# laurabragagnolo/SkelSplat

Measured on AMD Instinct MI355X. Metric: rendered+backpropagated views/s (differentiable skeletal-Gaussian rasterizer fwd+bwd), higher is better.
Workload: dtype f32

## Files before the change

### include/skelsplat_hip.h

```cpp
#ifndef SKELSPLAT_HIP_H
#define SKELSPLAT_HIP_H

#include <stddef.h>
#include <stdint.h>

#ifdef __cplusplus
extern "C" {
#endif

#define SKS_MAX_VIEWS 64
#define SKS_MAX_CHANNELS 32
#define SKS_SMALL_P 256

#define SKS_ANTIALIASING 1u
#define SKS_CLAMP01      2u
#define SKS_FORCE_BINNED 4u
#define SKS_DEBUG_SYNC   8u

#define SKS_NO_NT_STORES 16u

#define SKS_RAW_PARAMS   32u
#define SKS_RAW_GRADS    128u
#define SKS_BIN_CLEAN    64u
#define SKS_BIN_GROUPS_SHIFT 16
#define SKS_BIN_GROUPS(n) ((unsigned)(((n) - 1) & 7) << SKS_BIN_GROUPS_SHIFT)
#define SKS_FILL_LINEAR (1u << 21)
#define SKS_FILL_ROWS (1u << 22)
#define SKS_BWD_LDS_LIST (1u << 20)
#define SKS_BWD_WG_SHIFT 23

const char* sks_last_error(void);
int sks_version(void);

int sks_scratch_bytes(int V, int P, int C, int W, int H, size_t bin_capacity,
                      size_t* geom_bytes, size_t* binning_bytes, size_t* accum_bytes);

int sks_forward(int V, int P, int C, int W, int H,
                const float* viewmatrix, const float* projmatrix,
                const float* tanfovx , const float* tanfovy ,
                const float* means3D, const float* features, const float* opacities,
                const float* scales, const float* rotations, const float* cov3D_precomp,
                float scale_modifier, unsigned flags,
                float* out_color, float* out_invdepth, int* radii,
                void* geom, void* binning, size_t bin_capacity, int* num_rendered_dev,
                float* final_T, uint32_t* n_contrib, void* stream);

int sks_backward(int V, int P, int C, int W, int H,
                 const float* viewmatrix, const float* projmatrix,
                 const float* tanfovx , const float* tanfovy ,
                 const float* bg,
                 const float* means3D, const float* features, const float* opacities,
                 const float* scales, const float* rotations, const float* cov3D_precomp,
                 float scale_modifier, unsigned flags,
                 const int* radii, const void* geom, const void* binning, size_t bin_capacity,
                 const float* dL_dout_color, const float* dL_dout_invdepth,
                 void* accum,
                 float* dL_dmeans3D, float* dL_dmeans2D, float* dL_dopacity,
                 float* dL_dscales, float* dL_drotations, float* dL_dcov3D, float* dL_dfeatures,
                 float* dL_dmeans3D_mean ,
                 void* stream);

#define SKS_FB_NO_JOIN 1u
// ... 189 lines not shown
```

### skelsplat_amd/_lib.py

```python
import ctypes as C
import os

_HERE = os.path.dirname(os.path.abspath(__file__))
LIB_PATH = os.path.join(_HERE, "libskelsplat_hip.so")
_lib = None

SKS_MAX_VIEWS = 64
SKS_MAX_CHANNELS = 32
SKS_SMALL_P = 256
SKS_ANTIALIASING = 1
SKS_CLAMP01 = 2
SKS_FORCE_BINNED = 4
SKS_DEBUG_SYNC = 8
SKS_NO_NT_STORES = 16
SKS_RAW_PARAMS = 32
SKS_BIN_CLEAN = 64
SKS_RAW_GRADS = 128
SKS_FB_NO_JOIN = 1
SKS_BIN_GROUPS_SHIFT = 16
SKS_SSIM_SCRATCH_BYTES = 64 * 8
SKS_SOFTARGMAX_STATS = 6
SKS_REPORT_MAX_SAVES = 8
SKS_EVAL_MAX_GROUPS = 64


def SKS_BIN_GROUPS(n):
    return ((int(n) - 1) & 7) << SKS_BIN_GROUPS_SHIFT


_vp, _i, _u, _f, _sz = C.c_void_p, C.c_int, C.c_uint, C.c_float, C.c_size_t

_CAMERAS = (("V", _i), ("P", _i), ("C", _i), ("W", _i), ("H", _i), ("viewmatrix", _vp), ("projmatrix", _vp),
            ("tanfovx", _vp), ("tanfovy", _vp))
_GAUSSIANS = (("means3D", _vp), ("features", _vp), ("opacities", _vp), ("scales", _vp), ("rotations", _vp),
              ("cov3D_precomp", _vp), ("scale_modifier", _f), ("flags", _u))
_UPSTREAM = (("dL_dout_color", _vp), ("dL_dout_invdepth", _vp), ("accum", _vp))
_GRADS = (("dL_dmeans3D", _vp), ("dL_dmeans2D", _vp), ("dL_dopacity", _vp), ("dL_dscales", _vp), ("dL_drotations", _vp),
          ("dL_dcov3D", _vp), ("dL_dfeatures", _vp), ("dL_dmeans3D_mean", _vp))
_FORWARD_IO = (("out_color", _vp), ("out_invdepth", _vp), ("radii", _vp), ("geom", _vp), ("binning", _vp),
               ("bin_capacity", _sz), ("num_rendered_dev", _vp))
FORWARD_PARAMS = _CAMERAS + _GAUSSIANS + _FORWARD_IO + (("final_T", _vp), ("n_contrib", _vp), ("stream", _vp))
BACKWARD_PARAMS = _CAMERAS + (("bg", _vp),) + _GAUSSIANS + (("radii", _vp), ("geom", _vp), ("binning", _vp), ("bin_capacity", _sz)) \
    + _UPSTREAM + _GRADS + (("stream", _vp),)
FORWARD_BACKWARD_PARAMS = _CAMERAS + _GAUSSIANS + _FORWARD_IO + (("bg", _vp),) + _UPSTREAM + _GRADS \
    + (("stream", _vp), ("aux_stream", _vp), ("fb_flags", _u))

FWD, BWD, FWD_BWD = ({name: i for i, (name, _) in enumerate(params)}
                     for params in (FORWARD_PARAMS, BACKWARD_PARAMS, FORWARD_BACKWARD_PARAMS))
FWD_BWD_SOURCES = tuple(("fwd", FWD[n]) if n in FWD else ("bwd", BWD[n]) if n in BWD else None for n in FWD_BWD)

_ull = C.c_ulonglong
_VIEWS_DV = (("viewmatrix", _vp), ("projmatrix", _vp), ("views_dev", _vp))
RIG_SELECT_PARAMS = (("R", _i), ("V", _i), ("frames", _i), ("rig_ids", _vp), ("bank_viewmatrix", _vp), ("bank_projmatrix", _vp),
                     ("bank_tan", _vp), ("slot_wh", _vp), ("bank_proj", _vp), ("bank_sched", _vp), ("viewmatrix", _vp),
                     ("projmatrix", _vp), ("views_dev", _vp), ("proj", _vp), ("lr_sched_dev", _vp), ("error_word", _vp),
                     ("stream", _vp))
# ... 147 lines not shown
```

### skelsplat_amd/csrc/sks_common.inc

```
thread_local char g_err[512] = "";

int fail(int code, const char* fmt, ...)
{
    va_list ap;
    va_start(ap, fmt);
    vsnprintf(g_err, sizeof(g_err), fmt, ap);
    va_end(ap);
    return code;
}

#define HIP_TRY(expr)                                                                          \
    do {                                                                                       \
        hipError_t e_ = (expr);                                                                \
        if (e_ != hipSuccess) return fail((int)e_, "%s: %s", #expr, hipGetErrorString(e_));    \
    } while (0)

#define STAGE_CHECK(name)                                                                      \
    do {                                                                                       \
        HIP_TRY(hipGetLastError());                                                            \
        if (flags & SKS_DEBUG_SYNC) {                                                          \
            hipError_t e_ = hipStreamSynchronize(st);                                          \
            if (e_ != hipSuccess) return fail((int)e_, "stage %s: %s", name, hipGetErrorString(e_)); \
        }                                                                                      \
    } while (0)

constexpr int PROF_MAX = 16384;
struct ProfKind {
    hipEvent_t b[PROF_MAX], e[PROF_MAX];
    int created = 0, n = 0;
};
struct ProfState {
    bool on = false;
    int every = 1;
    int skip = 0;
    bool recorded = false;
    int seen[2] = { 0, 0 };
    ProfKind kind[2];
};
thread_local ProfState* tl_prof = nullptr;

struct ProfScope {
    ProfKind* k = nullptr;
    hipStream_t st;
    bool ext;
    ProfScope(int kind, hipStream_t s, bool ext_ = false) : st(s), ext(ext_)
    {
        ProfState* ps = tl_prof;
        if (!ps || !ps->on || ((ps->skip >> kind) & 1)) return;
        if (ps->seen[kind]++ % ps->every != 0) return;
        ProfKind& p = ps->kind[kind];
        if (p.n >= PROF_MAX) return;
        if (p.n >= p.created) {
            if (hipEventCreate(&p.b[p.created]) != hipSuccess || hipEventCreate(&p.e[p.created]) != hipSuccess) return;
            p.created++;
        }
        k = &p;
        if (ps->recorded) ext = false;
        if (!ext) (void)hipEventRecord(p.b[p.n], st);
    }
    hipEvent_t eb() const { return k->b[k->n]; }
    hipEvent_t ee() const { return k->e[k->n]; }
    ~ProfScope()
    {
        if (!k) return;
        if (!ext) (void)hipEventRecord(k->e[k->n], st);
        k->n++;
    }
};
#define SKS_LAUNCH(prof, kernel, grid, block, lds, stream, ...)                                                  \
    do {                                                                                                         \
        if ((prof).k) hipExtLaunchKernelGGL(kernel, grid, block, lds, stream, (prof).eb(), (prof).ee(), 0, __VA_ARGS__); \
        else hipLaunchKernelGGL(kernel, grid, block, lds, stream, __VA_ARGS__);                                  \
    } while (0)

constexpr int NACC = 8;
constexpr int BWD_SPLITS = 16;
constexpr int BWD_WG_PAIRS16 = 400;
constexpr int BWD_WG_PAIRS8 = 4096;

struct ViewTan {
    float x[SKS_MAX_VIEWS];
    float y[SKS_MAX_VIEWS];
    int w[SKS_MAX_VIEWS];
    int h[SKS_MAX_VIEWS];
};
struct ViewOff {
    unsigned long long off[SKS_MAX_VIEWS];
};
struct ViewTanDev {
    const float* x;
    const float* y;
    const int* w;
    const int* h;
    const double* sched;
};
inline ViewTanDev views_dev_from(const void* views_dev, const double* sched = nullptr)
{
    const ViewTan* t = (const ViewTan*)views_dev;
    return ViewTanDev{ t->x, t->y, t->w, t->h, sched };
}
inline bool fill_views(ViewTan& vt, ViewOff* vo, int V, int C, int W, int H, const float* tanfovx, const float* tanfovy,
                       const int* view_wh, const size_t* plane_off)
{
    for (int v = 0; v < V; v++) {
        vt.x[v] = tanfovx[v];
// ... 154 lines not shown
```

### skelsplat_amd/csrc/sks_fwd_small.inc

```
__device__ __forceinline__ float clamp01(float x) { return fminf(fmaxf(x, 0.0f), 1.0f); }

struct FwdArgs {
    int P, C, W, H;
    unsigned flags;
    Geom g;
    const float* features;
    float* out_color;
    float* out_invdepth;
    float* final_T;
    uint32_t* n_contrib;
    int tslots;
    unsigned cp1_magic;
    int ncomp;
    int cover_planes;
    unsigned w_magic;
};

inline int composite_slots(unsigned flags, int V, int P)
{
    const int t = (int)((flags >> 26) & 15u);
    return t ? t : ((long long)V * P <= 128 ? 4 : 8);
}

typedef float v4f __attribute__((ext_vector_type(4)));
// ... 5 lines not shown
__device__ __forceinline__ void store4(float* p, float a, float b, float c, float d)
{
    v4f v = { a, b, c, d };
    if (NT) __builtin_nontemporal_store(v, reinterpret_cast<v4f*>(p));
    else *reinterpret_cast<v4f*>(p) = v;
}
template <bool NT>
__device__ __forceinline__ void store2(float* p, float a, float b)
{
    v2f v = { a, b };
    if (NT) __builtin_nontemporal_store(v, reinterpret_cast<v2f*>(p));
    else *reinterpret_cast<v2f*>(p) = v;
}

template <int CG>
struct DynList {
    float2* xy;
    float4* co;
    float* invd;
    float* feat;
    unsigned long long* key;
    uint4* rect;
    __device__ DynList(char* base, int cap)
    {
        co = (float4*)base; base += (size_t)cap * 16;
        rect = (uint4*)base; base += (size_t)cap * 16;
        key = (unsigned long long*)base; base += (size_t)cap * 8;
        xy = (float2*)base; base += (size_t)cap * 8;
        invd = (float*)base; base += (size_t)cap * 4;
        feat = (float*)base;
    }
    static size_t bytes(int cap, int cg) { return (size_t)cap * (16 + 16 + 8 + 8 + 4 + 4 * (size_t)cg); }
};

template <int PPT, bool NT, bool HALF = false>
__device__ __forceinline__ void fwd_fill_role(const FwdArgs& a, unsigned cp1_magic, int q, int band, int zid, int gy, int pb,
                                              const uint32_t* __restrict__ cover)
{
    const int tid = threadIdx.x;
    const int P = a.P, C = a.C, W = a.W, H = a.H;
    const size_t HW = (size_t)H * W;
    const int v = (int)(((unsigned)zid * cp1_magic) >> 20);
    const int plane = zid - v * (C + 1);
    const bool is_inv = plane == C;
    const int cw = cover_cw(W);
    constexpr int PASS = 256 * PPT;
    const int rows = min(TILE, H - band * TILE);
    const int Nb = rows * W;
    const size_t band0 = (size_t)band * TILE * W;
    float* out = (is_inv ? a.out_invdepth + (size_t)v * HW : a.out_color + ((size_t)v * C + plane) * HW) + band0;
    const int shift = (int)((reinterpret_cast<uintptr_t>(out) >> 2) & 31u);
    const int base0 = q * PASS * pb + tid * PPT - shift;
    float* outT = (is_inv && a.final_T) ? a.final_T + (size_t)v * HW + band0 : nullptr;
    uint32_t* outN = (is_inv && a.n_contrib) ? a.n_contrib + (size_t)v * HW + band0 : nullptr;
    const uint32_t* __restrict__ cwp = cover;
    v4u c0 = { 0u, 0u, 0u, 0u }, c1 = { 0u, 0u, 0u, 0u };
    if (cover) {
        const int wo = __builtin_amdgcn_readfirstlane(((a.cover_planes ? zid : v) * gy + band) * cw);
        cwp = cover + wo;
        c0 = *reinterpret_cast<const v4u*>(cwp);
        if (cw > 4) c1 = *reinterpret_cast<const v4u*>(cwp + 4);
    }
    const bool any = c0.x != 0u;
    const unsigned w_magic = a.w_magic;
    auto mod_w = [&](int base) -> int {
        if (w_magic) return base - (int)__umulhi((unsigned)base, w_magic) * W;
        return base % W;
    };
    auto cover_word = [&](int wi) -> uint32_t {
        if (cw <= 4) return wi == 0 ? c0.y : wi == 1 ? c0.z : c0.w;
        if (cw <= 8) return wi == 0 ? c0.y : wi == 1 ? c0.z : wi == 2 ? c0.w : wi == 3 ? c1.x : wi == 4 ? c1.y : wi == 5 ? c1.z : c1.w;
        return cwp[1 + wi];
    };
    if (pb < 0) {
        const int pbr = -pb;
        const int chunks = (W + PASS - 1) / PASS;
        const int rb = q / chunks, chunk = q - rb * chunks;
        const int x = chunk * PASS + tid * PPT;
        if (x >= W) return;
        if (any) {
            const int tx = x >> 4;
            if ((cover_word(tx >> 5) >> (tx & 31)) & 1u) return;
        }
        const int r1 = min(rows, (rb + 1) * pbr);
        for (int r = rb * pbr; r < r1; r++) {
            const int base = r * W + x;
            store4<NT>(out + base, 0.0f, 0.0f, 0.0f, 0.0f);
            if (outT || outN) {
#pragma unroll
                for (int p = 0; p < PPT; p++) {
                    if (outT) outT[base + p] = 1.0f;
                    if (outN) outN[base + p] = 0u;
                }
            }
        }
        return;
    }
    const int npass = min(pb, 32);
    if (cover && !any) {
        for (int k = 0; k < npass; k++) {
            const int base = base0 + k * PASS;
            if (base >= Nb) break;
            if (base < 0) continue;
            if (PPT == 4) store4<NT>(out + base, 0.0f, 0.0f, 0.0f, 0.0f);
            else out[base] = 0.0f;
            if (outT || outN) {
#pragma unroll
                for (int p = 0; p < PPT; p++) {
                    if (outT) outT[base + p] = 1.0f;
                    if (outN) outN[base + p] = 0u;
                }
            }
        }
        return;
    }
    unsigned skipmask = 0u, skipmask2 = 0u;
    auto second_tx = [&](int x0) -> int { const int x1 = x0 + 2; return (x1 >= W ? x1 - W : x1) >> 4; };
    if (any && cw <= 8) {
        for (int k = 0; k < npass; k++) {
            const int base = base0 + k * PASS;
            if (base >= Nb) break;
            if (base < 0) continue;
            const int x0 = mod_w(base);
            const int tx = x0 >> 4;
            const bool s0 = (cover_word(tx >> 5) >> (tx & 31)) & 1u;
            bool s1 = s0;
            if (HALF) {
                const int tx1 = second_tx(x0);
                s1 = ((cover_word(tx1 >> 5) >> (tx1 & 31)) & 1u) || base + 2 >= Nb;
            }
            if (s0 && s1) continue;
            if (PPT == 4) {
                if (!HALF || (!s0 && !s1)) store4<NT>(out + base, 0.0f, 0.0f, 0.0f, 0.0f);
                else store2<NT>(out + base + (s0 ? 2 : 0), 0.0f, 0.0f);
            } else {
                out[base] = 0.0f;
            }
            if (outT || outN) {
#pragma unroll
                for (int p = 0; p < PPT; p++) {
                    if (HALF && (p < 2 ? s0 : s1)) continue;
                    if (outT) outT[base + p] = 1.0f;
                    if (outN) outN[base + p] = 0u;
                }
            }
        }
// ... 142 lines not shown
                    uint32_t contributor = 0, last = 0;
                    for (int k = 0; k < n; k++) {
                        contributor++;
                        const float2 xy = L.xy[k];
                        const float4 co = L.co[k];
                        const float dx = xy.x - pxf, dy = xy.y - pyf;
                        const float power = -0.5f * (co.x * dx * dx + co.z * dy * dy) - co.y * dx * dy;
                        if (power > 0.0f) continue;
                        const float alpha = fminf(0.99f, co.w * expf_fixed(power));
                        if (alpha < 1.0f / 255.0f) continue;
                        const float test_T = T * (1 - alpha);
                        if (test_T < 0.0001f) break;
#pragma unroll
                        for (int ch = 0; ch < CG; ch++) acc[ch] += L.feat[k * CG + ch] * alpha * T;
                        inv += L.invd[k] * alpha * T;
                        T = test_T;
                        last = contributor;
                    }
                    const size_t pix = (size_t)y * W + x;
#pragma unroll
                    for (int ch = 0; ch < CG; ch++)
                        if (ch < C && ((chm >> ch) & 1u)) outc[(size_t)ch * HW + pix] = do_clamp ? clamp01(acc[ch]) : acc[ch];
                    outi[pix] = inv;
                    if (a.final_T) a.final_T[(size_t)v * HW + pix] = T;
                    if (a.n_contrib) a.n_contrib[(size_t)v * HW + pix] = last;
                }
            }
            __syncthreads();
        }
        return;
    }
    fwd_fill_role<PPT, NT, HALF>(a, cp1_magic, xq, band_id, zid, gy, pb, cover);
}
```

### skelsplat_amd/csrc/sks_geom_fwd.inc

```
template <class VT>
__device__ __forceinline__ uint4 geom_fwd_one(int P, const VT& vt, const float* __restrict__ vms,
                                              const float* __restrict__ pms, const float* __restrict__ means,
                                              const float* __restrict__ opac, const float* __restrict__ scales,
                                              const float* __restrict__ rots, const float* __restrict__ cov3Dp,
                                              float smod, unsigned flags, const Geom& g, int* __restrict__ radii,
                                              int v, int idx, bool live, bool store = true)
{
    const size_t o = (size_t)v * P + (live ? idx : 0);
    const float* V = vms + 16 * v;
    const float* PM = pms + 16 * v;
    const float tan_fovx = vt.x[v], tan_fovy = vt.y[v];
    const int W = vt.w[v], H = vt.h[v];
    const float focal_y = H / (2.0f * tan_fovy);
    const float focal_x = W / (2.0f * tan_fovx);
    const int gx = (W + TILE - 1) / TILE, gy = (H + TILE - 1) / TILE;

    int radius_out = 0;
    uint4 rect = make_uint4(0, 0, 0, 0);
    float4 co = make_float4(0, 0, 0, 0), xyd = make_float4(0, 0, 1.0f, 1.0f);

    const int li = live ? idx : 0;
    const float p_orig[3] = { means[3 * li], means[3 * li + 1], means[3 * li + 2] };
    float p_view[3];
    transformPoint4x3(p_orig, V, p_view);
// ... 25 lines not shown
        const float det = det_cov_plus_h_cov;
        if (det != 0.0f) {
            const float det_inv = 1.f / det;
            const float conic[3] = { cov_z * det_inv, -cov_y * det_inv, cov_x * det_inv };
            const float mid = 0.5f * (cov_x + cov_z);
            const float lambda1 = mid + sqrtf(fmaxf(0.1f, mid * mid - det));
            const float lambda2 = mid - sqrtf(fmaxf(0.1f, mid * mid - det));
            const float my_radius = ceilf(3.f * sqrtf(fmaxf(lambda1, lambda2)));
            const float px = ndc2Pix(p_proj[0], W), py = ndc2Pix(p_proj[1], H);
            int xmin, ymin, xmax, ymax;
            getRect(px, py, (int)my_radius, gx, gy, xmin, ymin, xmax, ymax);
            if ((xmax - xmin) * (ymax - ymin) != 0) {
                radius_out = (int)my_radius;
                rect = make_uint4(xmin, ymin, xmax, ymax);
                const float op_raw = opac[li];
                const float op = (flags & SKS_RAW_PARAMS) ? 1.0f / (1.0f + expf_fixed(-op_raw)) : op_raw;
                co = make_float4(conic[0], conic[1], conic[2], op * h_convolution_scaling);
                xyd = make_float4(px, py, p_view[2], 1 / p_view[2]);
            }
        }
    }
    if (live && store) {
        radii[o] = radius_out;
        g.co[o] = co;
        g.xyd[o] = xyd;
        g.rect[o] = rect;
    }
    return rect;
}

#ifndef SKS_GEOM_COVER_THREADS
#define SKS_GEOM_COVER_THREADS 256
#endif
__global__ __launch_bounds__(SKS_GEOM_COVER_THREADS > 256 ? SKS_GEOM_COVER_THREADS : 256) void k_geom_fwd(int P, int W, int H, ViewTan vt, const float* __restrict__ vms,
                                                   const float* __restrict__ pms, const float* __restrict__ means,
                                                   const float* __restrict__ opac, const float* __restrict__ scales,
                                                   const float* __restrict__ rots, const float* __restrict__ cov3Dp,
                                                   float smod, unsigned flags, Geom g, int* __restrict__ radii, int vf,
                                                   uint32_t* __restrict__ count = nullptr, uint32_t* __restrict__ touched = nullptr,
                                                   const float* __restrict__ features = nullptr, int C = 0,
                                                   uint2* __restrict__ fmask = nullptr, uint32_t* __restrict__ bin_hdr = nullptr,
                                                   int cover_planes = 0)
{
    __shared__ uint32_t s_cov[COVER_MAX_WORDS];
    const int idx = blockIdx.x * blockDim.x + threadIdx.x;
    const int v = blockIdx.y;
    const bool live = idx < P;
    if (vf > 0) {
        const int fr = v / vf;
        means += (size_t)fr * P * 3;
        opac += (size_t)fr * P;
        if (scales) scales += (size_t)fr * P * 3;
        if (rots) rots += (size_t)fr * P * 4;
        if (cov3Dp) cov3Dp += (size_t)fr * P * 6;
    }
    const int pz = blockIdx.z;
    const uint4 rect = geom_fwd_one(P, vt, vms, pms, means, opac, scales, rots, cov3Dp, smod, flags, g, radii, v, idx, live, pz == 0);
    if (bin_hdr && blockIdx.x == 0 && blockIdx.y == 0 && pz == 0 && threadIdx.x < 64) bin_hdr[threadIdx.x] = 0u;
    if (count) {
        const int wt = (int)(rect.z - rect.x), n = wt * (int)(rect.w - rect.y);
        if (live) touched[(size_t)v * P + idx] = (uint32_t)n;
        if (live && v == 0) {
            unsigned fm = 0u;
            float f0 = 0.0f;
            for (int ch = C - 1; ch >= 0; ch--) {
                const float f = features[(size_t)idx * C + ch];
                if (f != 0.0f) { fm |= 1u << ch; f0 = f; }
            }
            fmask[idx] = make_uint2(fm, __float_as_uint(f0));
        }
    }
    if (g.cover) {
        const int gy = (H + TILE - 1) / TILE;
        const int cw = cover_cw(W), pw = gy * cw;
        for (int i = threadIdx.x; i < pw; i += blockDim.x) s_cov[i] = 0u;
        __syncthreads();
        bool mine = live && rect.z > rect.x && rect.w > rect.y;
        if (mine && cover_planes && pz < C) mine = features[(size_t)idx * C + pz] != 0.0f;
        if (mine) {
#pragma nounroll
            for (unsigned y = rect.y; y < rect.w; y++) {
                atomicOr(&s_cov[y * cw], 1u);
#pragma nounroll
                for (unsigned w0 = rect.x >> 5; w0 <= (rect.z - 1u) >> 5; w0++) {
                    const unsigned lo = max(rect.x, w0 << 5) & 31u, hi = min(rect.z - 1u, (w0 << 5) + 31u) & 31u;
                    atomicOr(&s_cov[y * cw + 1 + w0], (0xffffffffu >> (31u - hi)) & (0xffffffffu << lo));
                }
            }
        }
        __syncthreads();
        uint32_t* out = g.cover + ((size_t)v * (cover_planes ? C + 1 : 1) + (cover_planes ? pz : 0)) * pw;
        for (int i = threadIdx.x; i < pw; i += blockDim.x) out[i] = s_cov[i];
    }
}

__global__ __launch_bounds__(256) void k_geom_fwd_dv(int P, ViewTanDev vt, const float* __restrict__ vms, const float* __restrict__ pms,
                                                      const float* __restrict__ means, const float* __restrict__ opac,
                                                      const float* __restrict__ scales, const float* __restrict__ rots,
                                                      const float* __restrict__ cov3Dp, float smod, unsigned flags, Geom g,
                                                      int* __restrict__ radii, int vf)
{
    const int idx = blockIdx.x * 256 + threadIdx.x;
    const int v = blockIdx.y;
    if (vf > 0) {
        const int fr = v / vf;
        means += (size_t)fr * P * 3;
        opac += (size_t)fr * P;
        if (scales) scales += (size_t)fr * P * 3;
        if (rots) rots += (size_t)fr * P * 4;
        if (cov3Dp) cov3Dp += (size_t)fr * P * 6;
    }
    geom_fwd_one(P, vt, vms, pms, means, opac, scales, rots, cov3Dp, smod, flags, g, radii, v, idx, idx < P);
}

__global__ void k_mark_visible(int P, const float* __restrict__ means, const float* __restrict__ V,
                               uint8_t* __restrict__ present)
{
    const int idx = blockIdx.x * 256 + threadIdx.x;
    if (idx >= P) return;
    const float p[3] = { means[3 * idx], means[3 * idx + 1], means[3 * idx + 2] };
    float pv[3];
    transformPoint4x3(p, V, pv);
    present[idx] = pv[2] > 0.2f;
}
```

### skelsplat_amd/csrc/sks_raster.hip

```cpp
#include <hip/hip_runtime.h>
#include <hip/hip_ext.h>
#include <stdarg.h>
#include <stdlib.h>
#include <stdio.h>
#include <string.h>
#include <type_traits>

#include "../../include/skelsplat_hip.h"
#include "sks_math.h"
#include "sks_loop_dev.h"

using namespace sks;

namespace {

#include "sks_common.inc"
#include "sks_geom_fwd.inc"
#include "sks_fwd_small.inc"
#include "sks_bwd_small.inc"
#include "sks_geom_bwd.inc"
#include "sks_binned.inc"

inline int pick_cg(int C) { return C <= 4 ? 4 : C <= 16 ? 16 : C <= 20 ? 20 : 32; }

// ... 3 lines not shown
    if (P < 0) return fail(-1, "P=%d negative", P);
    if (C < 1 || C > SKS_MAX_CHANNELS) return fail(-1, "C=%d out of range [1,%d]", C, SKS_MAX_CHANNELS);
    if (W < 1 || H < 1 || W > 4096 * TILE || H > 65535 * TILE) return fail(-1, "image %dx%d out of range", W, H);
    return 0;
}

inline bool fill_half_mode(const FwdArgs& a) { return a.W % 4 == 2 && a.H % 2 == 0 && !(a.flags & SKS_NO_NT_STORES); }

inline void fill_geometry(const FwdArgs& a, bool have_cover, bool binned, int& fsplit, int& pb)
{
    const int ppt = (a.W % 4 == 0 || fill_half_mode(a)) ? 4 : 1;
    const bool lines = (((uintptr_t)a.out_color | (uintptr_t)a.out_invdepth) & 127u) == 0;
    const int lead = (lines && (long long)a.H * a.W % 32 == 0 && TILE * a.W % 32 == 0) ? 0 : 31;
    const int passes = (TILE * a.W + lead + 256 * ppt - 1) / (256 * ppt);
    const int tune = (int)((a.flags >> 8) & 0xff);
    const int chunks = (a.W + 1023) / 1024;
    const bool rowmode = ((ppt == 4 && a.W % 4 == 0 && have_cover && a.W % 32 == 0 && (long long)a.W * 10 >= (long long)chunks * 1024 * 9) ||
                          (ppt == 4 && a.W % 4 == 0 && have_cover && (a.flags & SKS_FILL_ROWS))) && !(a.flags & SKS_FILL_LINEAR);
    if (rowmode) {
        int pbr = tune;
        if (pbr <= 0) pbr = binned ? 3 : 2;
        if (pbr > TILE) pbr = TILE;
        fsplit = chunks * ((TILE + pbr - 1) / pbr);
        pb = -pbr;
        return;
    }
    pb = tune;
    if (pb <= 0) pb = passes / 8 > 2 ? (passes + 4) / 8 : 2;
    if (pb > 32) pb = 32;
    fsplit = (passes + pb - 1) / pb;
}

template <int CG>
void launch_fwd_small(const FwdArgs& a_in, int V, int gy, hipStream_t st, const ProfScope& prof)
{
    FwdArgs a = a_in;
    const int ncomp = a.tslots * a.P * V;
    a.ncomp = ncomp;
    int fsplit, pb;
    fill_geometry(a, a.g.cover != nullptr, false, fsplit, pb);
    const int rows_zy = (a.C + 1) * V * gy;
    const int xc = (ncomp + rows_zy - 1) / rows_zy;
    const int cap = (a.P + 15) & ~15;
    const size_t lds = DynList<CG>::bytes(cap, CG);
    dim3 grid(fsplit + xc, gy, (a.C + 1) * V);
    const bool nt = !(a.flags & SKS_NO_NT_STORES);
    if (a.W % 4 == 0) {
        if (nt) SKS_LAUNCH(prof, (k_render_fwd_sparse<CG, 4, true>), grid, dim3(256), lds, st, a, a.cp1_magic, gy, fsplit, pb, (const uint32_t*)a.g.cover);
        else SKS_LAUNCH(prof, (k_render_fwd_sparse<CG, 4, false>), grid, dim3(256), lds, st, a, a.cp1_magic, gy, fsplit, pb, (const uint32_t*)a.g.cover);
    } else if (fill_half_mode(a)) {
        SKS_LAUNCH(prof, (k_render_fwd_sparse<CG, 4, true, true>), grid, dim3(256), lds, st, a, a.cp1_magic, gy, fsplit, pb, (const uint32_t*)a.g.cover);
    } else {
        SKS_LAUNCH(prof, (k_render_fwd_sparse<CG, 1, false>), grid, dim3(256), lds, st, a, a.cp1_magic, gy, fsplit, pb, (const uint32_t*)a.g.cover);
    }
}

template <int CG>
void launch_fwd_binned(const FwdArgs& a, const BinView& bv, int V, int gx, int gy, const uint32_t* cover, hipStream_t st)
{
    int fsplit, pb;
    fill_geometry(a, true, true, fsplit, pb);
    const int xc = ((gx + TGROUP - 1) / TGROUP + a.C) / (a.C + 1);
    dim3 grid(fsplit + xc, gy, (a.C + 1) * V);
    const bool nt = !(a.flags & SKS_NO_NT_STORES);
    if (a.W % 4 == 0) {
        if (nt) hipLaunchKernelGGL((k_render_fwd_binned<CG, 4, true>), grid, dim3(256), 0, st, a, bv, gx, gy, fsplit, pb, cover);
        else hipLaunchKernelGGL((k_render_fwd_binned<CG, 4, false>), grid, dim3(256), 0, st, a, bv, gx, gy, fsplit, pb, cover);
    } else if (fill_half_mode(a)) {
        hipLaunchKernelGGL((k_render_fwd_binned<CG, 4, true, true>), grid, dim3(256), 0, st, a, bv, gx, gy, fsplit, pb, cover);
    } else {
        hipLaunchKernelGGL((k_render_fwd_binned<CG, 1, false>), grid, dim3(256), 0, st, a, bv, gx, gy, fsplit, pb, cover);
    }
}

inline int bwd_tile_blocks()
{
    static const int n = [] {
        int dev = 0, cus = 256;
        if (hipGetDevice(&dev) == hipSuccess) {
            hipDeviceProp_t pr;
            if (hipGetDeviceProperties(&pr, dev) == hipSuccess && pr.multiProcessorCount > 0) cus = pr.multiProcessorCount;
        }
        const char* e = getenv("SKS_BWD_TILE_BLOCKS");
        return (e && atoi(e) > 0) ? atoi(e) : cus * BWD_TILE_BLOCKS_PER_CU;
    }();
    return n;
}
// ... 133 lines not shown
                 void* stream, const FwdHook* hook)
{
    if (int rc = check_common(V, P, C, W, H)) return rc;
    hipStream_t st = (hipStream_t)stream;
    if (!out_color || !out_invdepth) return fail(-2, "out_color / out_invdepth must be provided");
    if (((uintptr_t)out_color | (uintptr_t)out_invdepth) & 15u)
        return fail(-2, "out_color / out_invdepth must be 16-byte aligned (the planes are written with 16-byte stores)");
    const size_t HW = (size_t)H * W;
    if (P == 0) {
        HIP_TRY(hipMemsetAsync(out_color, 0, (size_t)V * C * HW * 4, st));
        HIP_TRY(hipMemsetAsync(out_invdepth, 0, (size_t)V * HW * 4, st));
        if (final_T) return fail(-2, "final_T not available for P == 0");
        return 0;
    }
    if (!viewmatrix || !projmatrix || !tanfovx || !tanfovy || !means3D || !features || !opacities || !radii || !geom)
        return fail(-2, "missing required pointer");
    if (!cov3D_precomp && (!scales || !rotations)) return fail(-2, "need scales+rotations or cov3D_precomp");
    ViewTan vt;
    ViewOff vo;
    fill_views(vt, &vo, V, C, W, H, tanfovx, tanfovy, nullptr, nullptr);
    Geom g = geom_from(geom, V, P, W, H);
    const int gx = (W + TILE - 1) / TILE, gy = (H + TILE - 1) / TILE, NT = gx * gy;

    const bool small = P <= SKS_SMALL_P && !(flags & SKS_FORCE_BINNED);
    Bin b{};
    if (!small) {
        if (!binning) return fail(-2, "binned path needs a binning buffer");
        if (bin_capacity < 1) return fail(-1, "binned path needs bin_capacity >= 1");
        b = bin_from(binning, V, P, NT, bin_capacity);
    }
    if (!small) g.cover = nullptr;
    const int gthreads = small ? 256 : SKS_GEOM_BINNED_THREADS;
    const int gplanes = (small && g.cover && cover_per_plane(P, W, H, C)) ? C + 1 : 1;
    if (hook && small && hook->geom_done)
        hipExtLaunchKernelGGL(k_geom_fwd, dim3((P + gthreads - 1) / gthreads, V, gplanes), dim3(gthreads), 0, st, nullptr, hook->geom_done, 0,
                              P, W, H, vt, viewmatrix, projmatrix, means3D, opacities, scales, rotations, cov3D_precomp, scale_modifier,
                              flags, g, radii, 0, (uint32_t*)nullptr, (uint32_t*)nullptr, features, C, (uint2*)nullptr, (uint32_t*)nullptr,
                              cover_per_plane(P, W, H, C) ? 1 : 0);
    else
    hipLaunchKernelGGL(k_geom_fwd, dim3((P + gthreads - 1) / gthreads, V, gplanes), dim3(gthreads), 0, st, P, W, H, vt, viewmatrix, projmatrix,
                       means3D, opacities, scales, rotations, cov3D_precomp, scale_modifier, flags, g, radii, 0,
                       small ? (uint32_t*)nullptr : b.count, small ? (uint32_t*)nullptr : b.touched, features, C,
                       small ? (uint2*)nullptr : b.fmask, small ? (uint32_t*)nullptr : b.hdr, (small && cover_per_plane(P, W, H, C)) ? 1 : 0);
    STAGE_CHECK("geometry");
    if (hook && small && hook->after_geom) {
        if (int rc = hook->after_geom(hook->ctx)) return rc;
    }

    FwdArgs a{ P, C, W, H, flags, g, features, out_color, out_invdepth, final_T, n_contrib, composite_slots(flags, V, P),
               ((1u << 20) + (unsigned)C) / (unsigned)(C + 1), 0, (!small || (g.cover && cover_per_plane(P, W, H, C))) ? 1 : 0,
               (W >= 2 && W < 16384) ? (unsigned)(((1ull << 32) + (unsigned)W - 1) / (unsigned)W) : 0u };
    const int cg = pick_cg(C);
    if (small) {
        {
            ProfScope prof(0, st, true);
            switch (cg) {
                case 4: launch_fwd_small<4>(a, V, gy, st, prof); break;
                case 16: launch_fwd_small<16>(a, V, gy, st, prof); break;
                case 20: launch_fwd_small<20>(a, V, gy, st, prof); break;
                default: launch_fwd_small<32>(a, V, gy, st, prof); break;
            }
        }
        STAGE_CHECK("render(small)");
        return 0;
    }
    uint32_t* cover = b.coverp;
    const int cw = cover_cw(W);
    hipLaunchKernelGGL(k_bin_band_count, dim3(gy, V), dim3(BAND_TC), (size_t)2 * gx * 4, st, P, gx, g, b);
    int vg, ng;
    bin_groups(flags, V, vg, ng);
    {
        const int bpc = gx >= SCAN_T * 8 ? 1 : (SCAN_T * 8) / gx;
        const int nchunk_t = (gy + bpc - 1) / bpc, nchunk_g = (P + SCAN_G - 1) / SCAN_G;
        hipLaunchKernelGGL(k_bin_scan, dim3(nchunk_t + nchunk_g, V), dim3(SCAN_T), (size_t)bpc * cw * 4, st, P, gx, gy, cw, bpc,
                           nchunk_t, bin_capacity, b, cover, num_rendered_dev, V, C + 1, vg);
    }
    hipLaunchKernelGGL(k_bin_band_scatter, dim3(gy, V), dim3(BAND_TS), (size_t)2 * gx * 4, st, P, gx, bin_capacity, g, b, C, cw);
    STAGE_CHECK("binning");
    const BinView bv_all = bin_view(b, NT, bin_capacity);
    {
        ProfScope prof(0, st);
        for (int gi = 0; gi < ng; gi++) {
            const int v0 = gi * vg, nv = (V - v0 < vg) ? V - v0 : vg;
            FwdArgs ag = a;
            ag.out_color = a.out_color + (size_t)v0 * C * HW;
            ag.out_invdepth = a.out_invdepth + (size_t)v0 * HW;
            if (a.final_T) ag.final_T = a.final_T + (size_t)v0 * HW;
            if (a.n_contrib) ag.n_contrib = a.n_contrib + (size_t)v0 * HW;
            BinView bv = bv_all;
            bv.ranges += (size_t)v0 * NT;
            bv.tidx += (size_t)v0 * NT;
            bv.aux += (size_t)v0 * NT * TILE * TILE;
            bv.e_co += (size_t)v0 * bin_capacity;
// ... 150 lines not shown
    int vg = V, ng = 1;
    if (!small && V >= 1) bin_groups(flags, V, vg, ng);
    struct Ctx {
        int V, P, C, W, H;
        const float *vm, *pm, *tx, *ty, *bg, *means, *feat, *opac, *scales, *rots, *cov;
        float smod;
        unsigned flags;
        const int* radii;
        const void *geom, *binning;
        size_t cap;
        const float *dL, *dLinv;
        void* accum;
        float *m3, *m2, *op, *sc, *rot, *dcov, *dfeat, *mean;
        hipStream_t s, aux;
        bool ext, handed;
        int rc_aux;
        int backward(unsigned phases, int group) const
        {
            return backward_impl(V, P, C, W, H, vm, pm, tx, ty, bg, means, feat, opac, scales, rots, cov, smod, flags, radii, geom, binning, cap,
                                 dL, dLinv, accum, m3, m2, op, sc, rot, dcov, dfeat, mean, aux, phases, group);
        }
    } c{ V, P, C, W, H, viewmatrix, projmatrix, tanfovx, tanfovy, bg, means3D, features, opacities, scales, rotations, cov3D_precomp,
         scale_modifier, flags, radii, geom, binning, bin_capacity, dL_dout_color, dL_dout_invdepth, accum, dL_dmeans3D, dL_dmeans2D,
         dL_dopacity, dL_dscales, dL_drotations, dL_dcov3D, dL_dfeatures, dL_dmeans3D_mean, (hipStream_t)stream, (hipStream_t)aux_stream,
         true, false, 0 };
    {
        static const bool ext_off = [] { const char* e = getenv("SKS_FB_EXT"); return e && atoi(e) == 0; }();
        if (ext_off) c.ext = false;
    }
    const bool no_join = (fb_flags & SKS_FB_NO_JOIN) != 0;
    const bool crowded = small && (long long)V * P > FB_OVERLAP_MAX_PAIRS && !no_join;
    if (!aux_stream || aux_stream == stream || P == 0 || (flags & SKS_DEBUG_SYNC) || (!small && ng < 2) || crowded) {
        if (int rc = forward_impl(V, P, C, W, H, viewmatrix, projmatrix, tanfovx, tanfovy, means3D, features, opacities, scales, rotations,
                                  cov3D_precomp, scale_modifier, flags, out_color, out_invdepth, radii, geom, binning, bin_capacity,
                                  num_rendered_dev, nullptr, nullptr, stream, nullptr))
            return rc;
        if (int rc = backward_impl(V, P, C, W, H, viewmatrix, projmatrix, tanfovx, tanfovy, bg, means3D, features, opacities, scales,
                                   rotations, cov3D_precomp, scale_modifier, flags, radii, geom, binning, bin_capacity, dL_dout_color,
                                   dL_dout_invdepth, accum, dL_dmeans3D, dL_dmeans2D, dL_dopacity, dL_dscales, dL_drotations, dL_dcov3D,
                                   dL_dfeatures, dL_dmeans3D_mean, stream, BWD_RENDER | BWD_GEOM, -1))
            return rc;
        if (no_join && aux_stream && aux_stream != stream) {
            FbEvents* ev = nullptr;
            if (int rc = fb_events(0, ev)) return rc;
            HIP_TRY(hipEventRecord(ev->done, (hipStream_t)stream));
            HIP_TRY(hipStreamWaitEvent((hipStream_t)aux_stream, ev->done, 0));
        }
        return 0;
    }
    FbEvents* evp = nullptr;
    if (int rc = fb_events(small ? 0 : ng, evp)) return rc;
    FbEvents& ev = *evp;
    struct Run {
        static int after_geom(void* p)
        {
            Ctx& k = *(Ctx*)p;
            FbEvents& e = tl_fb_events;
            if (!k.ext) HIP_TRY(hipEventRecord(e.geom, k.s));
            HIP_TRY(hipStreamWaitEvent(k.aux, e.geom, 0));
            k.handed = true;
            return k.rc_aux = k.backward(BWD_RENDER | BWD_GEOM, -1);
        }
        static int after_group(void* p, int g, int, int)
        {
            Ctx& k = *(Ctx*)p;
            FbEvents& e = tl_fb_events;
            HIP_TRY(hipEventRecord(e.grp[g], k.s));
// ... 368 lines not shown
```

Measured before the change: 60360.

## Fuse geometry pass with early fill of trailing output planes in small forward

Adds a combined kernel in which the first blocks run per-Gaussian geometry and the rest zero-fill a tail of output planes. This lets the fill stores overlap with geometry work, and the following render launch then covers only the remaining planes. It targets the serial gap and launch cost between geometry and the fill/render stage. It adds flag-bit reuse, magic-number index division and profiling-event plumbing, and it is disabled on the combined fwd+bwd path without an aux stream.

```diff
diff --git a/include/skelsplat_hip.h b/include/skelsplat_hip.h
--- a/include/skelsplat_hip.h
+++ b/include/skelsplat_hip.h
@@ -28,6 +28,8 @@
 #define SKS_FILL_ROWS (1u << 22)
 #define SKS_BWD_LDS_LIST (1u << 20)
 #define SKS_BWD_WG_SHIFT 23
+#define SKS_NO_EARLY_FILL (1u << 30)
+#define SKS_EARLY_FILL(n) (((unsigned)(n) & 7u) << SKS_BIN_GROUPS_SHIFT)
 
 const char* sks_last_error(void);
 int sks_version(void);
diff --git a/skelsplat_amd/_lib.py b/skelsplat_amd/_lib.py
--- a/skelsplat_amd/_lib.py
+++ b/skelsplat_amd/_lib.py
@@ -22,6 +22,13 @@
 SKS_SOFTARGMAX_STATS = 6
 SKS_REPORT_MAX_SAVES = 8
 SKS_EVAL_MAX_GROUPS = 64
+
+
+SKS_NO_EARLY_FILL = 1 << 30
+
+
+def SKS_EARLY_FILL(n):
+    return (int(n) & 7) << SKS_BIN_GROUPS_SHIFT
 
 
 def SKS_BIN_GROUPS(n):
diff --git a/skelsplat_amd/csrc/sks_common.inc b/skelsplat_amd/csrc/sks_common.inc
--- a/skelsplat_amd/csrc/sks_common.inc
+++ b/skelsplat_amd/csrc/sks_common.inc
@@ -43,6 +43,7 @@
     ProfKind* k = nullptr;
     hipStream_t st;
     bool ext;
+    bool began = false;
     ProfScope(int kind, hipStream_t s, bool ext_ = false) : st(s), ext(ext_)
     {
         ProfState* ps = tl_prof;
@@ -69,8 +70,15 @@
 };
 #define SKS_LAUNCH(prof, kernel, grid, block, lds, stream, ...)                                                  \
     do {                                                                                                         \
-        if ((prof).k) hipExtLaunchKernelGGL(kernel, grid, block, lds, stream, (prof).eb(), (prof).ee(), 0, __VA_ARGS__); \
+        if ((prof).k)                                                                                            \
+            hipExtLaunchKernelGGL(kernel, grid, block, lds, stream, (prof).began ? nullptr : (prof).eb(), (prof).ee(), 0, __VA_ARGS__); \
         else hipLaunchKernelGGL(kernel, grid, block, lds, stream, __VA_ARGS__);                                  \
+    } while (0)
+#define SKS_LAUNCH_FIRST(prof, kernel, grid, block, lds, stream, ...)                                            \
+    do {                                                                                                         \
+        if ((prof).k && (prof).ext) hipExtLaunchKernelGGL(kernel, grid, block, lds, stream, (prof).eb(), nullptr, 0, __VA_ARGS__); \
+        else hipLaunchKernelGGL(kernel, grid, block, lds, stream, __VA_ARGS__);    \
+        (prof).began = (prof).k != nullptr;                                                                      \
     } while (0)
 
 constexpr int NACC = 8;
diff --git a/skelsplat_amd/csrc/sks_fwd_small.inc b/skelsplat_amd/csrc/sks_fwd_small.inc
--- a/skelsplat_amd/csrc/sks_fwd_small.inc
+++ b/skelsplat_amd/csrc/sks_fwd_small.inc
@@ -61,6 +61,26 @@
     }
     static size_t bytes(int cap, int cg) { return (size_t)cap * (16 + 16 + 8 + 8 + 4 + 4 * (size_t)cg); }
 };
+
+template <int PPT, bool NT>
+__device__ __forceinline__ void fill_bare(float* out, float* outT, uint32_t* outN, int base0, int Nb, int npass)
+{
+    constexpr int PASS = 256 * PPT;
+    for (int k = 0; k < npass; k++) {
+        const int base = base0 + k * PASS;
+        if (base >= Nb) break;
+        if (base < 0) continue;
+        if (PPT == 4) store4<NT>(out + base, 0.0f, 0.0f, 0.0f, 0.0f);
+        else out[base] = 0.0f;
+        if (outT || outN) {
+#pragma unroll
+            for (int p = 0; p < PPT; p++) {
+                if (outT) outT[base + p] = 1.0f;
+                if (outN) outN[base + p] = 0u;
+            }
+        }
+    }
+}
 
 template <int PPT, bool NT, bool HALF = false>
 __device__ __forceinline__ void fwd_fill_role(const FwdArgs& a, unsigned cp1_magic, int q, int band, int zid, int gy, int pb,
@@ -127,20 +147,7 @@
     }
     const int npass = min(pb, 32);
     if (cover && !any) {
-        for (int k = 0; k < npass; k++) {
-            const int base = base0 + k * PASS;
-            if (base >= Nb) break;
-            if (base < 0) continue;
-            if (PPT == 4) store4<NT>(out + base, 0.0f, 0.0f, 0.0f, 0.0f);
-            else out[base] = 0.0f;
-            if (outT || outN) {
-#pragma unroll
-                for (int p = 0; p < PPT; p++) {
-                    if (outT) outT[base + p] = 1.0f;
-                    if (outN) outN[base + p] = 0u;
-                }
-            }
-        }
+        fill_bare<PPT, NT>(out, outT, outN, base0, Nb, npass);
         return;
     }
     unsigned skipmask = 0u, skipmask2 = 0u;
@@ -349,3 +356,48 @@
     }
     fwd_fill_role<PPT, NT, HALF>(a, cp1_magic, xq, band_id, zid, gy, pb, cover);
 }
+
+struct EarlyFill {
+    float* out_color;
+    float* out_invdepth;
+    int C, W, H, gy;
+    int gplanes;
+    int ngeom;
+    int zid0;
+    int fsplit, pb;
+    unsigned cp1_magic;
+    unsigned row_magic;
+    unsigned fs_magic;
+};
+
+template <int PPT, bool NT>
+__global__ __launch_bounds__(256) void k_geom_fwd_fill(EarlyFill f, int P, ViewTan vt, const float* __restrict__ vms,
+                                                       const float* __restrict__ pms, const float* __restrict__ means,
+                                                       const float* __restrict__ opac, const float* __restrict__ scales,
+                                                       const float* __restrict__ rots, const float* __restrict__ cov3Dp, float smod,
+                                                       unsigned flags, Geom g, int* __restrict__ radii,
+                                                       const float* __restrict__ features, int cover_planes)
+{
+    const int b = blockIdx.x;
+    if (b < f.ngeom) {
+        const int v = f.gplanes == 1 ? b : (int)(((unsigned)b * f.cp1_magic) >> 20);
+        extern __shared__ __attribute__((aligned(16))) char s_dyn[];
+        geom_fwd_block((uint32_t*)s_dyn, 0, v, b - v * f.gplanes, P, f.W, f.H, vt, vms, pms, means, opac, scales, rots, cov3Dp, smod, flags, g, radii, 0,
+                       nullptr, nullptr, features, f.C, nullptr, nullptr, cover_planes);
+        return;
+    }
+    const unsigned e = (unsigned)(b - f.ngeom);
+    const unsigned rows = (unsigned)(f.fsplit * f.gy);
+    const unsigned zr = f.row_magic ? __umulhi(e, f.row_magic) : e;
+    const unsigned rem = e - zr * rows;
+    const int band = (int)(f.fs_magic ? __umulhi(rem, f.fs_magic) : rem);
+    const int q = (int)rem - band * f.fsplit;
+    const int zid = f.zid0 + (int)zr;
+    const int v = (int)(((unsigned)zid * f.cp1_magic) >> 20);
+    const int plane = zid - v * (f.C + 1);
+    const size_t HW = (size_t)f.H * f.W;
+    const int Nb = min(TILE, f.H - band * TILE) * f.W;
+    float* out = (plane == f.C ? f.out_invdepth + (size_t)v * HW : f.out_color + ((size_t)v * f.C + plane) * HW) + (size_t)band * TILE * f.W;
+    const int shift = (int)((reinterpret_cast<uintptr_t>(out) >> 2) & 31u);
+    fill_bare<PPT, NT>(out, nullptr, nullptr, q * (256 * PPT) * f.pb + (int)threadIdx.x * PPT - shift, Nb, min(f.pb, 32));
+}
diff --git a/skelsplat_amd/csrc/sks_geom_fwd.inc b/skelsplat_amd/csrc/sks_geom_fwd.inc
--- a/skelsplat_amd/csrc/sks_geom_fwd.inc
+++ b/skelsplat_amd/csrc/sks_geom_fwd.inc
@@ -81,19 +81,16 @@
 #ifndef SKS_GEOM_COVER_THREADS
 #define SKS_GEOM_COVER_THREADS 256
 #endif
-__global__ __launch_bounds__(SKS_GEOM_COVER_THREADS > 256 ? SKS_GEOM_COVER_THREADS : 256) void k_geom_fwd(int P, int W, int H, ViewTan vt, const float* __restrict__ vms,
-                                                   const float* __restrict__ pms, const float* __restrict__ means,
-                                                   const float* __restrict__ opac, const float* __restrict__ scales,
-                                                   const float* __restrict__ rots, const float* __restrict__ cov3Dp,
-                                                   float smod, unsigned flags, Geom g, int* __restrict__ radii, int vf,
-                                                   uint32_t* __restrict__ count = nullptr, uint32_t* __restrict__ touched = nullptr,
-                                                   const float* __restrict__ features = nullptr, int C = 0,
-                                                   uint2* __restrict__ fmask = nullptr, uint32_t* __restrict__ bin_hdr = nullptr,
-                                                   int cover_planes = 0)
+__device__ __forceinline__ void geom_fwd_block(uint32_t* s_cov, int bx, int v, int pz, int P, int W, int H, const ViewTan& vt, const float* __restrict__ vms,
+                                               const float* __restrict__ pms, const float* __restrict__ means,
+                                               const float* __restrict__ opac, const float* __restrict__ scales,
+                                               const float* __restrict__ rots, const float* __restrict__ cov3Dp,
+                                               float smod, unsigned flags, const Geom& g, int* __restrict__ radii, int vf,
+                                               uint32_t* __restrict__ count, uint32_t* __restrict__ touched,
+                                               const float* __restrict__ features, int C,
+                                               uint2* __restrict__ fmask, uint32_t* __restrict__ bin_hdr, int cover_planes)
 {
-    __shared__ uint32_t s_cov[COVER_MAX_WORDS];
-    const int idx = blockIdx.x * blockDim.x + threadIdx.x;
-    const int v = blockIdx.y;
+    const int idx = bx * blockDim.x + threadIdx.x;
     const bool live = idx < P;
     if (vf > 0) {
         const int fr = v / vf;
@@ -103,9 +100,8 @@
         if (rots) rots += (size_t)fr * P * 4;
         if (cov3Dp) cov3Dp += (size_t)fr * P * 6;
     }
-    const int pz = blockIdx.z;
     const uint4 rect = geom_fwd_one(P, vt, vms, pms, means, opac, scales, rots, cov3Dp, smod, flags, g, radii, v, idx, live, pz == 0);
-    if (bin_hdr && blockIdx.x == 0 && blockIdx.y == 0 && pz == 0 && threadIdx.x < 64) bin_hdr[threadIdx.x] = 0u;
+    if (bin_hdr && bx == 0 && v == 0 && pz == 0 && threadIdx.x < 64) bin_hdr[threadIdx.x] = 0u;
     if (count) {
         const int wt = (int)(rect.z - rect.x), n = wt * (int)(rect.w - rect.y);
         if (live) touched[(size_t)v * P + idx] = (uint32_t)n;
@@ -143,6 +139,21 @@
     }
 }
 
+__global__ __launch_bounds__(SKS_GEOM_COVER_THREADS > 256 ? SKS_GEOM_COVER_THREADS : 256) void k_geom_fwd(int P, int W, int H, ViewTan vt, const float* __restrict__ vms,
+                                                   const float* __restrict__ pms, const float* __restrict__ means,
+                                                   const float* __restrict__ opac, const float* __restrict__ scales,
+                                                   const float* __restrict__ rots, const float* __restrict__ cov3Dp,
+                                                   float smod, unsigned flags, Geom g, int* __restrict__ radii, int vf,
+                                                   uint32_t* __restrict__ count = nullptr, uint32_t* __restrict__ touched = nullptr,
+                                                   const float* __restrict__ features = nullptr, int C = 0,
+                                                   uint2* __restrict__ fmask = nullptr, uint32_t* __restrict__ bin_hdr = nullptr,
+                                                   int cover_planes = 0)
+{
+    __shared__ uint32_t s_cov[COVER_MAX_WORDS];
+    geom_fwd_block(s_cov, blockIdx.x, blockIdx.y, blockIdx.z, P, W, H, vt, vms, pms, means, opac, scales, rots, cov3Dp, smod, flags, g, radii, vf,
+                   count, touched, features, C, fmask, bin_hdr, cover_planes);
+}
+
 __global__ __launch_bounds__(256) void k_geom_fwd_dv(int P, ViewTanDev vt, const float* __restrict__ vms, const float* __restrict__ pms,
                                                       const float* __restrict__ means, const float* __restrict__ opac,
                                                       const float* __restrict__ scales, const float* __restrict__ rots,
diff --git a/skelsplat_amd/csrc/sks_raster.hip b/skelsplat_amd/csrc/sks_raster.hip
--- a/skelsplat_amd/csrc/sks_raster.hip
+++ b/skelsplat_amd/csrc/sks_raster.hip
@@ -59,18 +59,19 @@
 }
 
 template <int CG>
-void launch_fwd_small(const FwdArgs& a_in, int V, int gy, hipStream_t st, const ProfScope& prof)
+void launch_fwd_small(const FwdArgs& a_in, int V, int gy, int zfill, hipStream_t st, const ProfScope& prof)
 {
     FwdArgs a = a_in;
     const int ncomp = a.tslots * a.P * V;
     a.ncomp = ncomp;
     int fsplit, pb;
     fill_geometry(a, a.g.cover != nullptr, false, fsplit, pb);
-    const int rows_zy = (a.C + 1) * V * gy;
+    if (zfill == 0) fsplit = 0;
+    const int rows_zy = (zfill > 0 ? zfill : 1) * gy;
     const int xc = (ncomp + rows_zy - 1) / rows_zy;
     const int cap = (a.P + 15) & ~15;
     const size_t lds = DynList<CG>::bytes(cap, CG);
-    dim3 grid(fsplit + xc, gy, (a.C + 1) * V);
+    dim3 grid(fsplit + xc, gy, zfill > 0 ? zfill : 1);
     const bool nt = !(a.flags & SKS_NO_NT_STORES);
     if (a.W % 4 == 0) {
         if (nt) SKS_LAUNCH(prof, (k_render_fwd_sparse<CG, 4, true>), grid, dim3(256), lds, st, a, a.cp1_magic, gy, fsplit, pb, (const uint32_t*)a.g.cover);
@@ -80,6 +81,49 @@
     } else {
         SKS_LAUNCH(prof, (k_render_fwd_sparse<CG, 1, false>), grid, dim3(256), lds, st, a, a.cp1_magic, gy, fsplit, pb, (const uint32_t*)a.g.cover);
     }
+}
+
+#ifndef SKS_EARLY_FILL_BYTES
+#define SKS_EARLY_FILL_BYTES (36u << 20)
+#endif
+inline int early_fill_planes(unsigned flags, int planes, size_t plane_bytes)
+{
+    const int field = (int)((flags >> SKS_BIN_GROUPS_SHIFT) & 7u);
+    if (field == 7) return planes;
+    if (field) return (planes * field + 15) / 16;
+    const size_t want = ((size_t)SKS_EARLY_FILL_BYTES + plane_bytes / 2) / plane_bytes;
+    return (int)(want < (size_t)(planes / 4) ? want : (size_t)(planes / 4));
+}
+
+inline unsigned magic32(unsigned d) { return (unsigned)(((1ull << 32) + d - 1) / d); }
+
+bool early_fill_cut(const FwdArgs& a_in, int V, int gy, int gplanes, int zid0, int& fsplit, int& pb)
+{
+    FwdArgs a = a_in;
+    a.flags |= SKS_FILL_LINEAR;
+    fill_geometry(a, true, false, fsplit, pb);
+    const long long rows = (long long)fsplit * gy, nfill = rows * ((a.C + 1) * V - zid0);
+    return fsplit >= 1 && pb >= 1 && nfill * rows < (1ll << 32) && (long long)V * gplanes + nfill < (1ll << 31);
+}
+
+void launch_geom_fill(const FwdArgs& a, int V, int gy, int gplanes, int zid0, int fsplit, int pb, const ViewTan& vt,
+                      const float* viewmatrix, const float* projmatrix, const float* means3D, const float* opacities,
+                      const float* scales, const float* rotations, const float* cov3D_precomp, float smod, int* radii,
+                      hipStream_t st, ProfScope& prof)
+{
+    const long long rows = (long long)fsplit * gy, nfill = rows * ((a.C + 1) * V - zid0);
+    const int ngeom = V * gplanes;
+    const EarlyFill f{ a.out_color, a.out_invdepth, a.C, a.W, a.H, gy, gplanes, ngeom, zid0, fsplit, pb, a.cp1_magic,
+                       rows > 1 ? magic32((unsigned)rows) : 0u, fsplit > 1 ? magic32((unsigned)fsplit) : 0u };
+    const dim3 grid((unsigned)(ngeom + nfill));
+    const size_t lds = (size_t)gy * cover_cw(a.W) * 4;
+    const bool nt = !(a.flags & SKS_NO_NT_STORES);
+    const int ppt = (a.W % 4 == 0 || fill_half_mode(a)) ? 4 : 1;
+#define SKS_GF_ARGS f, a.P, vt, viewmatrix, projmatrix, means3D, opacities, scales, rotations, cov3D_precomp, smod, a.flags, a.g, radii, a.features, a.cover_planes
+    if (ppt == 4 && nt) SKS_LAUNCH_FIRST(prof, (k_geom_fwd_fill<4, true>), grid, dim3(256), lds, st, SKS_GF_ARGS);
+    else if (ppt == 4) SKS_LAUNCH_FIRST(prof, (k_geom_fwd_fill<4, false>), grid, dim3(256), lds, st, SKS_GF_ARGS);
+    else SKS_LAUNCH_FIRST(prof, (k_geom_fwd_fill<1, false>), grid, dim3(256), lds, st, SKS_GF_ARGS);
+#undef SKS_GF_ARGS
 }
 
 template <int CG>
@@ -279,6 +323,28 @@
     if (!small) g.cover = nullptr;
     const int gthreads = small ? 256 : SKS_GEOM_BINNED_THREADS;
     const int gplanes = (small && g.cover && cover_per_plane(P, W, H, C)) ? C + 1 : 1;
+    FwdArgs a{ P, C, W, H, flags, g, features, out_color, out_invdepth, final_T, n_contrib, composite_slots(flags, V, P),
+               ((1u << 20) + (unsigned)C) / (unsigned)(C + 1), 0, (!small || (g.cover && cover_per_plane(P, W, H, C))) ? 1 : 0,
+               (W >= 2 && W < 16384) ? (unsigned)(((1ull << 32) + (unsigned)W - 1) / (unsigned)W) : 0u };
+    const int cg = pick_cg(C);
+    const int planes = (C + 1) * V;
+    int early = 0;
+    if (small && !hook && g.cover && !final_T && !n_contrib && !(flags & (SKS_DEBUG_SYNC | SKS_NO_EARLY_FILL)))
+        early = early_fill_planes(flags, planes, HW * 4);
+    int efs = 0, epb = 0;
+    if (early > 0 && early_fill_cut(a, V, gy, gplanes, planes - early, efs, epb)) {
+        ProfScope prof(0, st, true);
+        launch_geom_fill(a, V, gy, gplanes, planes - early, efs, epb, vt, viewmatrix, projmatrix, means3D, opacities, scales, rotations,
+                         cov3D_precomp, scale_modifier, radii, st, prof);
+        switch (cg) {
+            case 4: launch_fwd_small<4>(a, V, gy, planes - early, st, prof); break;
+            case 16: launch_fwd_small<16>(a, V, gy, planes - early, st, prof); break;
+            case 20: launch_fwd_small<20>(a, V, gy, planes - early, st, prof); break;
+            default: launch_fwd_small<32>(a, V, gy, planes - early, st, prof); break;
+        }
+        HIP_TRY(hipGetLastError());
+        return 0;
+    }
     if (hook && small && hook->geom_done)
         hipExtLaunchKernelGGL(k_geom_fwd, dim3((P + gthreads - 1) / gthreads, V, gplanes), dim3(gthreads), 0, st, nullptr, hook->geom_done, 0,
                               P, W, H, vt, viewmatrix, projmatrix, means3D, opacities, scales, rotations, cov3D_precomp, scale_modifier,
@@ -294,18 +360,14 @@
         if (int rc = hook->after_geom(hook->ctx)) return rc;
     }
 
-    FwdArgs a{ P, C, W, H, flags, g, features, out_color, out_invdepth, final_T, n_contrib, composite_slots(flags, V, P),
-               ((1u << 20) + (unsigned)C) / (unsigned)(C + 1), 0, (!small || (g.cover && cover_per_plane(P, W, H, C))) ? 1 : 0,
-               (W >= 2 && W < 16384) ? (unsigned)(((1ull << 32) + (unsigned)W - 1) / (unsigned)W) : 0u };
-    const int cg = pick_cg(C);
     if (small) {
         {
             ProfScope prof(0, st, true);
             switch (cg) {
-                case 4: launch_fwd_small<4>(a, V, gy, st, prof); break;
-                case 16: launch_fwd_small<16>(a, V, gy, st, prof); break;
-                case 20: launch_fwd_small<20>(a, V, gy, st, prof); break;
-                default: launch_fwd_small<32>(a, V, gy, st, prof); break;
+                case 4: launch_fwd_small<4>(a, V, gy, planes, st, prof); break;
+                case 16: launch_fwd_small<16>(a, V, gy, planes, st, prof); break;
+                case 20: launch_fwd_small<20>(a, V, gy, planes, st, prof); break;
+                default: launch_fwd_small<32>(a, V, gy, planes, st, prof); break;
             }
         }
         STAGE_CHECK("render(small)");
@@ -522,7 +584,7 @@
     const bool crowded = small && (long long)V * P > FB_OVERLAP_MAX_PAIRS && !no_join;
     if (!aux_stream || aux_stream == stream || P == 0 || (flags & SKS_DEBUG_SYNC) || (!small && ng < 2) || crowded) {
         if (int rc = forward_impl(V, P, C, W, H, viewmatrix, projmatrix, tanfovx, tanfovy, means3D, features, opacities, scales, rotations,
-                                  cov3D_precomp, scale_modifier, flags, out_color, out_invdepth, radii, geom, binning, bin_capacity,
+                                  cov3D_precomp, scale_modifier, flags | SKS_NO_EARLY_FILL, out_color, out_invdepth, radii, geom, binning, bin_capacity,
                                   num_rendered_dev, nullptr, nullptr, stream, nullptr))
             return rc;
         if (int rc = backward_impl(V, P, C, W, H, viewmatrix, projmatrix, tanfovx, tanfovy, bg, means3D, features, opacities, scales,
```

New measurement: 63250, median of 6. 1.05x the previous value.
